# magneano/shyft

Measured on NVIDIA B200. Metric: cell-timesteps/sec (pt_gs_k run_cells), higher is better.
Workload: dtype f64

## Files before the change

### shyft_b200/csrc/sb2_capi.cu

```cuda
#include <cuda_runtime.h>

#include <cstdio>
#include <cstdlib>
#include <cstring>
#include <map>
#include <mutex>
#include <memory>
#include <string>
#include <type_traits>
#include <vector>

#include "../../include/shyft_b200.h"
#include "sb2_host.hpp"
#include "sb2_interp.cuh"
#include "sb2_ptgsk.cuh"
#include "sb2_hbv.cuh"
#include "sb2_ptssk.cuh"
#include "sb2_pthpsk.cuh"
#include "sb2_routing.cuh"
#include <nvtx3/nvToolsExt.h>
#include "sb2_unit.cuh"
#include "sb2_goal.cuh"
#include "sb2_stats.cuh"

// ... 209 lines not shown
};

inline int grid_for(int64_t n, int block) { return int((n + block - 1) / block); }

}

#define SB2_HBV_UNIT_STEPS 64
#define SB2_DENSE_TILE_COMPACT 32

struct sb2_model {
    int stack = 0, device = 0;
    cudaStream_t stream = 0;
    std::string err;
    int64_t n = 0;
    std::vector<sb2_geo_cell> geo;
    std::vector<int64_t> cix_of_cell, cix_to_cid;
    std::map<int64_t, int64_t> cid_to_cix;
    int n_param = 0, n_state = 0;
    std::vector<double> region_param;
    std::map<int64_t, std::vector<double>> catch_param;
    bool param_dirty = true;
    std::vector<uint8_t> catchment_filter;
    bool filter_dirty = true;
    DevArray<double> d_x, d_y, d_z, d_area, d_glacier, d_lake, d_reservoir, d_forest, d_slope;
    DevArray<int32_t> d_pset;
    DevArray<uint8_t> d_active;
    DevArray<PtgskParam> d_ptgsk_params;
    DevArray<HbvParam> d_hbv_params;
    DevArray<SskParam> d_ssk_params;
    DevArray<HpsParam> d_hps_params;
    DevArray<double> d_state, d_initial_state;
    bool has_initial = false;
    int64_t t0 = 0, dt = 0, T = 0;
    DevArray<int2> d_doy_soy;
    std::vector<double> h_prior_gradient;
    DevArray<double> d_prior_gradient;
    DevArray<double> d_forcing[SB2_N_FORCING];
    int64_t forcing_first = 0, forcing_rows = 0;
    Source src[SB2_N_FORCING];
    sb2_interpolation_parameter ip{};
    bool ip_valid = false;
    IdwPlan idw[SB2_N_FORCING];
    std::vector<std::unique_ptr<BtkOps>> btk_cache;
    DevArray<double> d_btk_kbuf, d_btk_beta, d_btk_resid;
    bool force_sparse_idw = false;
    int collect_bits = SB2_COLLECT_DISCHARGE;
    DevArray<double> d_resp[SB2_N_RESPONSE], d_st[SB2_N_STATE_SERIES];
    int64_t out_first = 0, out_rows = 0;
    int64_t ran_first = 0, ran_steps = 0;
    DevArray<double> d_cq, d_cc;
    DevArray<int32_t> d_slot, d_cat_ptr, d_cat_slots;
    int64_t n_slots = 0;
    DevArray<double> d_partial;
    DevArray<double> d_scr[5];
    DevArray<int> d_tickets;
    int partial_steps = 0;
    DevArray<int> d_error_flag, d_scan_flag;
    std::vector<double> rivers;
    std::unique_ptr<RoutingPlan> route;
    DevArray<double> d_rlocal, d_rup, d_rout;
    bool rlocal_valid = false, rnet_valid = false;
    DevArray<double> d_qhist;
    int64_t qhist_rows = 0;
    struct Target {
        std::vector<double> obs;
        int64_t t0 = 0, dt = 0;
        std::vector<int64_t> cids;
        int64_t river_id = 0;
        double scale_factor = 1.0;
        int calc_mode = 0, property = 0;
        double s_r = 1.0, s_a = 1.0, s_b = 1.0;
        DevArray<double> d_obs, d_series;
        DevArray<int32_t> d_cix;
        bool aligned = true;
        std::vector<int64_t> points;
        DevArray<int64_t> d_points;
        DevArray<double> d_projected, d_scale;
    };
    std::vector<std::unique_ptr<Target>> targets;
    DevArray<int32_t> d_cell_ptr, d_cell_of_catch;
    DevArray<int64_t> d_axis_t;
    DevArray<int32_t> d_one_zero;
    int64_t launches = 0;
    float last_step_ms = 0.f, last_interp_ms = 0.f;
    cudaEvent_t ev[4] = {nullptr, nullptr, nullptr, nullptr};

    int64_t n_catch() const { return int64_t(cix_to_cid.size()); }
    void use_device() const { CUDA_OK(cudaSetDevice(device)); }
};

namespace {

template <class F>
int guarded(sb2_model* m, F&& f) {
    try {
        if (!m) throw Error("null model");
        m->use_device();
        f();
        return 0;
    } catch (const std::exception& e) {
        if (m) m->err = e.what();
        return 1;
    }
}
template <class F>
int guarded_c(const sb2_model* m, F&& f) { return guarded(const_cast<sb2_model*>(m), f); }

// ... 133 lines not shown
    const PtgskParam* ptgsk_members = nullptr;
    const HbvParam* hbv_members = nullptr;
    const HpsParam* hps_members = nullptr;
    double* state = nullptr;
    double* partial = nullptr;
    double *cq = nullptr, *cc = nullptr;
    DevArray<double>* scr = nullptr;
    int64_t state_stride = 0, partial_stride = 0, catch_stride = 0, scr_stride = 0;
    int* tickets = nullptr;
    bool series = false;
};

void launch_step_chunk(sb2_model* m, const StepTarget& t, int64_t s0, int chunk, bool collect_end_state) {
    const int64_t n = m->n;
    const unsigned ne = unsigned(t.members);
    const bool gsk = m->stack == SB2_PT_GS_K;
    const int collect = t.series ? m->collect_bits : 0;
    const bool upar = m->catch_param.empty() && !t.ptgsk_members && !t.hbv_members && !t.hps_members;
    const int groups = step_groups(m);
    const bool split = use_time_split(int64_t(groups) * t.members);
    const int unit_steps = split ? (gsk ? SB2_UNIT_STEPS : SB2_HBV_UNIT_STEPS) : 0;
    const int n_slices = split ? grid_for(chunk, unit_steps) : 1;
    auto zero_tickets = [&] {
        if (split) CUDA_OK(cudaMemsetAsync(t.tickets, 0, size_t(t.members) * (1 + groups) * sizeof(int), m->stream));
    };
    auto common = [&](auto& a) {
        const double dt_seconds = double(m->dt) / 1e6;
        a.n_cells = n;
        a.area = m->d_area.p; a.glacier = m->d_glacier.p; a.lake = m->d_lake.p; a.reservoir = m->d_reservoir.p;
        a.pset = m->d_pset.p; a.active = m->d_active.p; a.state = t.state;
        for (int v = 0; v < 5; ++v) a.f[v] = m->d_forcing[v].p + (s0 - m->forcing_first) * n;
        a.n_steps = chunk; a.first_step = s0;
        a.dt_seconds = dt_seconds; a.dt_hours = dt_seconds / 3600.0; a.dt_us = double(m->dt);
        fill_dopri_products(a.dt_hours, a.dtb);
        if (t.series) {
            for (size_t r = 0; r < std::size(a.resp); ++r) a.resp[r] = m->d_resp[r].p;
            for (size_t s = 0; s < std::size(a.st); ++s) a.st[s] = m->d_st[s].p;
            a.out_first_step = m->out_first;
        }
        a.collect_end_state = collect_end_state ? 1 : 0;
        a.slot = m->d_slot.p; a.partial = t.partial; a.n_slots = m->n_slots; a.error_flag = m->d_error_flag.p;
        a.unit_steps = unit_steps; a.tickets = t.tickets; a.progress = t.tickets + t.members;
    };
    if (gsk) {
        PtgskRunArgs a{};
        common(a);
        a.z = m->d_z.p; a.forest = m->d_forest.p; a.params = m->d_ptgsk_params.p;
        a.bb0 = 0.98 * 5.670373e-8 * sb_pow4(273.15);
        a.inv_dt_seconds = make_inv_divisor(a.dt_seconds);
        a.inv_dt_us = make_inv_divisor(a.dt_us);
        a.par0 = make_ptgsk_param(m->region_param.data(), param_dt(m));
        a.day_sec_of_year = m->d_doy_soy.p;
        a.ens_params = t.ptgsk_members; a.ens_state_stride = t.state_stride; a.ens_partial_stride = t.partial_stride;
        for (int k = 0; k < 5; ++k) a.scr[k] = t.scr[k].p;
        a.ens_scr_stride = t.scr_stride;
        const dim3 ga((unsigned)grid_for(n, SB2_BLOCK_A), (unsigned)grid_for(chunk, SB2_STEPS_A), ne);
        const dim3 gb((unsigned)(grid_for(n, SB2_BLOCK_B) * n_slices), ne), gc((unsigned)(grid_for(n, SB2_BLOCK_C) * n_slices), ne);
        nvtxRangePushA("A forcing_terms");
        if (upar) ptgsk_forcing_terms_kernel<true><<<ga, SB2_BLOCK_A, SB2_MTAB_BYTES, m->stream>>>(a);
        else ptgsk_forcing_terms_kernel<false><<<ga, SB2_BLOCK_A, SB2_MTAB_BYTES, m->stream>>>(a);
        nvtxRangePop();
        zero_tickets();
        nvtxRangePushA("B snow");
        switch (collect & 14) {
#define SB2_CASE(B) case B: if (upar) ptgsk_snow_kernel<B, true><<<gb, SB2_BLOCK_B, SB2_MTAB_BYTES, m->stream>>>(a); \
                            else ptgsk_snow_kernel<B, false><<<gb, SB2_BLOCK_B, SB2_MTAB_BYTES, m->stream>>>(a); break;
            SB2_CASE(0) SB2_CASE(2) SB2_CASE(4) SB2_CASE(6) SB2_CASE(8) SB2_CASE(10) SB2_CASE(12) SB2_CASE(14)
#undef SB2_CASE
        }
        nvtxRangePop();
        zero_tickets();
        nvtxRangePushA("C response");
        switch (collect & 13) {
#define SB2_CASE(B) case B: if (upar) ptgsk_response_kernel<B, true><<<gc, SB2_BLOCK_C, SB2_MTAB_BYTES, m->stream>>>(a); \
                            else ptgsk_response_kernel<B, false><<<gc, SB2_BLOCK_C, SB2_MTAB_BYTES, m->stream>>>(a); break;
            SB2_CASE(0) SB2_CASE(1) SB2_CASE(4) SB2_CASE(5) SB2_CASE(8) SB2_CASE(9) SB2_CASE(12) SB2_CASE(13)
#undef SB2_CASE
        }
        nvtxRangePop();
        m->launches += 3;
    } else {
        const dim3 grid((unsigned)(groups * n_slices), ne);
        zero_tickets();
        if (m->stack == SB2_PT_SS_K) {
            SskRunArgs a{};
            common(a);
            a.params = m->d_ssk_params.p;
            a.inv_dt_hours = make_inv_divisor(a.dt_hours);
            a.step_in_days = a.dt_seconds / 86400.0;
            a.collect = collect & 15;
            ptssk_run_kernel<<<grid, SB2_BLOCK, SB2_MTAB_BYTES, m->stream>>>(a);
        } else if (m->stack == SB2_PT_HPS_K) {
            HpsRunArgs a{};
            common(a);
            a.params = m->d_hps_params.p;
            a.bb0 = 0.98 * 5.670373e-8 * sb_pow4(273.15);
            a.inv_dt_seconds = make_inv_divisor(a.dt_seconds);
            a.ens_params = t.hps_members; a.ens_state_stride = t.state_stride; a.ens_partial_stride = t.partial_stride;
            a.collect = collect & 15;
            if (t.hps_members) pthpsk_run_kernel<true><<<grid, SB2_BLOCK, SB2_MTAB_BYTES, m->stream>>>(a);
            else pthpsk_run_kernel<false><<<grid, SB2_BLOCK, SB2_MTAB_BYTES, m->stream>>>(a);
        } else {
            HbvRunArgs a{};
            common(a);
            a.params = m->d_hbv_params.p;
            a.inv_dt_hours = make_inv_divisor(a.dt_hours);
            a.step_in_days = a.dt_seconds / 86400.0;
// ... 482 lines not shown
            const int r = t.property == SB2_TARGET_SNOW_COVERED_AREA ? SB2_R_SNOW_SCA : SB2_R_SNOW_SWE;
            if (!m->d_resp[r].p || m->out_first != 0 || m->out_rows != m->T) throw Error(r == SB2_R_SNOW_SCA ? "resource collector doesn't have snow_sca" : "resource collector doesn't have snow_swe");
            std::vector<int32_t> cells;
            for (int64_t i = 0; i < m->n; ++i)
                for (auto cid : t.cids)
                    if (m->geo[i].catchment_id == cid) { cells.push_back(int32_t(i)); break; }
            std::vector<int32_t> ptr{0, int32_t(cells.size())};
            DevArray<int32_t> d_ptr, d_cells;
            d_ptr.upload(ptr, m->stream);
            d_cells.upload(cells, m->stream);
            t.d_series.resize(size_t(m->T));
            catchment_area_mean_kernel<<<grid_for(m->T, 256), 256, 0, m->stream>>>(m->d_resp[r].p, m->d_area.p, d_ptr.p, d_cells.p, 1, m->T, m->n,
                                                                                  t.d_series.p);
            CUDA_OK(cudaGetLastError());
            ++m->launches;
            CUDA_OK(cudaStreamSynchronize(m->stream));
        } else if (t.property == SB2_TARGET_ROUTED_DISCHARGE) {
            std::vector<double> out(size_t(m->T));
            if (sb2_river_flows(m, t.river_id, 0, m->T, nullptr, nullptr, out.data()) != 0) throw Error(m->err);
            t.d_series.upload(out, m->stream);
            CUDA_OK(cudaStreamSynchronize(m->stream));
        }
    }
}

double evaluate_goal_single(sb2_model* m) {
    prepare_snow_and_routed_targets(m);
    std::vector<GoalTarget> gt;
    build_goal_targets(m, gt, m->d_cq.p, m->d_cc.p, 0);
    DevArray<GoalTarget> d_gt;
    DevArray<double> d_out;
    d_gt.upload(gt, m->stream);
    d_out.resize(gt.size());
    goal_kernel<<<dim3((unsigned)gt.size(), 1), 256, 0, m->stream>>>(d_gt.p, int(gt.size()), d_out.p);
    CUDA_OK(cudaGetLastError());
    ++m->launches;
    std::vector<double> partial(gt.size());
    CUDA_OK(cudaMemcpyAsync(partial.data(), d_out.p, partial.size() * sizeof(double), cudaMemcpyDeviceToHost, m->stream));
    CUDA_OK(cudaStreamSynchronize(m->stream));
    return combine_goal(m, partial.data());
}

void goal_batch(sb2_model* m, int64_t n_sets, const double* P, double* goals) {
    sync_parameters(m);
    sync_filter(m);
    const bool gsk = m->stack == SB2_PT_GS_K;
    const int64_t n = m->n, T = m->T, nc = m->n_catch();
    const size_t state_sz = size_t(m->n_state) * n;
    const size_t per_member = state_sz * 8 + size_t(T) * nc * 16;
    const int64_t E = std::max<int64_t>(1, std::min<int64_t>(std::min<int64_t>(n_sets, 65535), int64_t((12ULL << 30) / per_member)));
    int64_t ps = std::min<int64_t>(T, int64_t((1ULL << 30) / (size_t(E) * m->n_slots * 16)));
    if (gsk) ps = std::min<int64_t>(ps, std::max<int64_t>(8, int64_t((4ULL << 30) / (size_t(E) * n * 40))));
    ps = std::max<int64_t>(1, ps);
    DevArray<double> d_state, d_partial, d_cq, d_cc, d_out, d_scr[5];
    if (gsk)
        for (auto& b : d_scr) b.resize(size_t(E) * ps * n);
    DevArray<int> d_tickets;
    d_tickets.resize(size_t(E) * (1 + step_groups(m)));
    DevArray<PtgskParam> d_par;
    DevArray<HbvParam> d_hbv_par;
    DevArray<HpsParam> d_hps_par;
    DevArray<GoalTarget> d_gt;
    d_state.resize(size_t(E) * state_sz);
    d_partial.resize(size_t(E) * ps * m->n_slots * 2);
    d_cq.resize(size_t(E) * T * nc);
    d_cc.resize(size_t(E) * T * nc);
    d_out.resize(size_t(E) * m->targets.size());
    std::vector<GoalTarget> gt;
    build_goal_targets(m, gt, d_cq.p, d_cc.p, T * nc);
    d_gt.upload(gt, m->stream);
    StepTarget t;
    t.state = d_state.p; t.partial = d_partial.p; t.cq = d_cq.p; t.cc = d_cc.p; t.scr = d_scr;
    t.state_stride = int64_t(state_sz); t.partial_stride = ps * m->n_slots * 2; t.catch_stride = T * nc; t.scr_stride = ps * n;
    t.tickets = d_tickets.p;
    std::vector<double> partial(size_t(E) * gt.size());
    for (int64_t e0 = 0; e0 < n_sets; e0 += E) {
        const int64_t ne = std::min<int64_t>(E, n_sets - e0);
        std::vector<const double*> sets;
        for (int64_t e = 0; e < ne; ++e) sets.push_back(P + (e0 + e) * m->n_param);
        if (gsk) { upload_params(m, sets, d_par); t.ptgsk_members = d_par.p; }
        else if (m->stack == SB2_PT_HPS_K) { upload_params(m, sets, d_hps_par); t.hps_members = d_hps_par.p; }
        else { upload_params(m, sets, d_hbv_par); t.hbv_members = d_hbv_par.p; }
        t.members = int(ne);
        for (int64_t e = 0; e < ne; ++e)
            CUDA_OK(cudaMemcpyAsync(d_state.p + e * state_sz, m->d_initial_state.p, state_sz * sizeof(double), cudaMemcpyDeviceToDevice, m->stream));
        for (int64_t done = 0; done < T; done += ps) launch_step_chunk(m, t, done, int(std::min<int64_t>(ps, T - done)), false);
        goal_kernel<<<dim3((unsigned)gt.size(), (unsigned)ne), 256, 0, m->stream>>>(d_gt.p, int(gt.size()), d_out.p);
        CUDA_OK(cudaGetLastError());
        ++m->launches;
        CUDA_OK(cudaMemcpyAsync(partial.data(), d_out.p, size_t(ne) * gt.size() * sizeof(double), cudaMemcpyDeviceToHost, m->stream));
        CUDA_OK(cudaStreamSynchronize(m->stream));
        for (int64_t e = 0; e < ne; ++e) goals[e0 + e] = combine_goal(m, partial.data() + e * gt.size());
    }
    check_device_errors(m);
}

std::vector<uint8_t> stat_selection(const sb2_model* m, const int64_t* indexes, int n_indexes, int scope) {
    if (m->n == 0) throw Error("no cells to make statistics on");
    std::vector<uint8_t> sel(size_t(m->n), n_indexes == 0 ? 1 : 0);
    if (n_indexes == 0) return sel;
    if (!indexes) throw Error("null index list");
    if (scope == SB2_SCOPE_CELL_IX) {
        for (int k = 0; k < n_indexes; ++k) {
            const int64_t cid = indexes[k];
            if (cid < 0 || cid > m->n)
                throw Error("Supplied cell index reference " + std::to_string(cid) + " is ouside valid range 0 .." + std::to_string(m->n));
            if (cid < m->n) sel[size_t(cid)] = 1;
// ... 1175 lines not shown
```

### shyft_b200/csrc/sb2_ptgsk.cuh

```cuda
#pragma once
#include <stdint.h>

#include "sb2_math.cuh"

namespace sb2 {

struct PtgskParam {
    double c1, c2, c3;
    double ae_scale_factor;
    double tx, wind_scale, max_water, wind_const, fast_albedo_decay_rate, slow_albedo_decay_rate, surface_magnitude, max_albedo,
        min_albedo, snowfall_reset_depth, snow_cv, glacier_albedo;
    double p_corr_scale_factor;
    double snow_cv_forest_factor, snow_cv_altitude_factor;
    double pt_albedo, pt_alpha;
    double initial_bare_ground_fraction;
    double gm_dtf, gm_direct_response;
    double reservoir_direct_response_fraction;
    double slow_albedo_decay_step;
    double fast_albedo_decay_step;
    int32_t winter_end_day_of_year;
    int32_t n_winter_days;
    int32_t calculate_iso_pot_energy;
    int32_t pad_;
    InvDivisor inv_snowfall_reset_depth, inv_one_minus_y0, inv_max_water, inv_ae_scale;
};

enum : int { ERR_KIRCHNER_STEP = 1 };

struct PtgskRunArgs {
    int64_t n_cells;
    const double* __restrict__ z;
    const double* __restrict__ area;
    const double* __restrict__ glacier;
    const double* __restrict__ lake;
    const double* __restrict__ reservoir;
    const double* __restrict__ forest;
    const int32_t* __restrict__ pset;
    const uint8_t* __restrict__ active;
    const PtgskParam* __restrict__ params;
    double* __restrict__ state;
    const double* __restrict__ f[5];
    int n_steps;
    int64_t first_step;
    double dt_seconds;
    double dt_hours;
    double dt_us;
    double bb0;
    InvDivisor inv_dt_seconds, inv_dt_us;
    double dtb[26];
    PtgskParam par0;
    const int2* __restrict__ day_sec_of_year;
    double* __restrict__ resp[8];
    double* __restrict__ st[9];
    int64_t out_first_step;
    int collect_end_state;
    const int32_t* __restrict__ slot;
    double* __restrict__ partial;
    int64_t n_slots;
    int* __restrict__ error_flag;
    const PtgskParam* __restrict__ ens_params;
    int64_t ens_state_stride, ens_partial_stride;
    double* __restrict__ scr[5];
    int64_t ens_scr_stride;
    int unit_steps;
    int* __restrict__ tickets;
    int* __restrict__ progress;
};
enum : int { SCR_POT = 0, SCR_LW = 1, SCR_TADD = 2, SCR_OUTFLOW = 3, SCR_SCA = 4 };

#define SB2_BLOCK 32

struct GsState { double albedo, lwc, surface_heat, alpha, sdc_melt_mean, acc_melt, iso_pot_energy, temp_swe; };
struct GsCache {
    double k_alpha, k_scale, k_acc, k_lwc, k_tswe;
    double storage, sca;
    double lg_key, lg_val;
};
__device__ __forceinline__ void gs_cache_clear(GsCache& c) {
    c.k_alpha = nan_(); c.lg_key = nan_();
    c.k_scale = c.k_acc = c.k_lwc = c.k_tswe = 0.0;
    c.storage = c.sca = c.lg_val = 0.0;
}
__device__ __forceinline__ bool gs_cache_hit(GsCache& c, double alpha, double scale, double acc, double lwc, double tswe) {
    return alpha == c.k_alpha && scale == c.k_scale && acc == c.k_acc && lwc == c.k_lwc && tswe == c.k_tswe;
}
__device__ __forceinline__ void gs_cache_store(GsCache& c, double alpha, double scale, double acc, double lwc, double tswe, double storage, double sca) {
    c.k_alpha = alpha; c.k_scale = scale; c.k_acc = acc; c.k_lwc = lwc; c.k_tswe = tswe;
    c.storage = storage; c.sca = sca;
}

enum : int { K_VP_A = 0, K_VP_B, K_VP_C, K_VP_D, K_VP_E, K_VP_F, K_VP_G, K_VP_H, K_LW, K_LW_EXP, K_SST_A, K_SST_B, K_TURB_A, K_TURB_B, K_TURB_C,
             K_SURF_A, K_SURF_B, K_KELVIN, K_PT_CK1, K_PT_PSYCR, K_PT_BOLZ, K_PT_CK2_NEG, K_PT_CK2_POS, K_PT_CK3_NEG, K_PT_CK3_POS, K_PT_EATM_A,
             K_PT_EATM_EXP, K_PT_EATM_B, K_PT_EMIS, K_MMH_M3S, K_TOL, K_EPS_ABS, K_EPS_REL, K_Q_MIN, K_GM, K_PHYS_N };
__constant__ double kPhysC[K_PHYS_N] = {33.864, 7.38e-3, 0.8072, 1.9e-5, 1.8, 1.316e-3, 9.72e-3, 4.2e-5, 0.98 * 5.670373e-8, 6.87e-2, 1.16, 2.09, 1.7, 6.12, 6.132,
                                        0.103, 0.186, 273.15, 0.610780, 0.066, 0.0000000567, 17.84362, 17.08085, 245.425, 234.175, 1.24,
                                        0.143, 0.85, 0.98, 1 / (3600.0 * 1000.0), 1.0e-10, 1.0e-7, 1.0e-8, 0.00001, 0.001 / 86400.0};
#define SB2_K(name) kPhysC[name]
__device__ __forceinline__ double mmh_to_m3s(double mmh, double area) { return area * mmh * SB2_K(K_MMH_M3S); }
__device__ __forceinline__ double m3s_to_mmh(double m3s, double area) { return m3s / (SB2_K(K_MMH_M3S) * area); }

__device__ __forceinline__ double gs_calc_q(double a, double b, double z, double lg_a, double lg_a1) {
    const double x = z / b;
    return a * b * gamma_p<true>(a + 1.0, x, lg_a1) + z * (1.0 - gamma_p<true>(a, x, lg_a));
}

__device__ __noinline__ double gs_corr_lwc(double z1, double a1, double b1, double a2, double b2) {
    const double Q1 = gs_calc_q(a1, b1, z1, sb_lgamma<true>(a1), sb_lgamma<true>(a1 + 1.0));
    const double lg_a2 = sb_lgamma<true>(a2), lg_a21 = sb_lgamma<true>(a2 + 1.0);
    auto f = [&](double z) {
        const double x = z / b2;
        double p1 = 0.0, p0 = 0.0;
        if (x == inf_()) p1 = p0 = 1.0;
        else if (x > 0.0) {
            const double lx = sb_log<true>(x);
            const double pre1 = sb_exp<true>((a2 + 1.0) * lx - x - lg_a21), pre0 = sb_exp<true>(a2 * lx - x - lg_a2);
            p1 = gamma_p_with_prefix(a2 + 1.0, x, pre1);
            p0 = gamma_p_with_prefix(a2, x, pre0);
        }
        const double d = (a2 * b2 * p1 + z * (1.0 - p0)) - Q1;
        return d * d;
    };
// ... 59 lines not shown
    if (lambda <= 0.0) {
        swe = m;
        sca = 1.0 - y0;
    } else if (lambda / scale > 1.3 * shape + 20.0) {
        swe = sca = 0.0;
        return;
    } else {
        const double x = lambda / scale;
        if (shape != lg_key) { lg_key = shape; lg_val = sb_lgamma<true>(shape); }
        lg = lg_val;
        have_lg = true;
        const double pre = gamma_prefix<true>(shape, x, lg);
        y = (x > 0.0) ? gamma_p_with_prefix(shape, x, pre) : 0.0;
        y1 = y - pre / shape;
        swe = m * (1.0 - y1) - lambda * (1 - y);
        sca = (1.0 - y) * (1.0 - y0);
    }
    if (lwd > m) swe *= 1.0 + max_water_frac;
    else if (lwd > 0.0) {
        const double sat = div_by(lwd, inv_mwf);
        const double x = sat / scale;
        if (!have_lg) {
            if (shape != lg_key) { lg_key = shape; lg_val = sb_lgamma<true>(shape); }
            lg = lg_val;
        }
        const double pre = gamma_prefix<true>(shape, x, lg);
        const double ssa = (x == inf_()) ? 1.0 : gamma_p_with_prefix(shape, x, pre);
        const double ssa1 = ssa - pre / shape;
        const double liqwat = max_water_frac * (m * (ssa1 - y1) + sat * (1.0 - ssa) - lambda * (1.0 - y));
        swe += liqwat;
    }
    swe += temp_swe;
    swe *= 1.0 - y0;
}

__device__ __forceinline__ void gs_reset_snow_pack(double& sca, double& lwc, double& alpha, double& sdc_melt_mean, double& acc_melt,
                                                   double& temp_swe, double storage, const PtgskParam& p) {
    if (storage > 1.0e-10) {
        sca = 1.0 - p.initial_bare_ground_fraction;
        sdc_melt_mean = storage / sca;
    } else {
        sca = sdc_melt_mean = 0.0;
    }
    alpha = 1.0 / (p.snow_cv * p.snow_cv);
    temp_swe = lwc = 0.0;
    acc_melt = -1.0;
}

__device__ __forceinline__ double gs_vapour_pressure(double T, double rel_hum) {
    double vapour_pressure = SB2_K(K_VP_A) * (sb_pow8(SB2_K(K_VP_B) * T + SB2_K(K_VP_C)) - SB2_K(K_VP_D) * fabs(SB2_K(K_VP_E) * T + 48.0) + SB2_K(K_VP_F)) * rel_hum;
    if (T < 0.0) vapour_pressure *= 1.0 + SB2_K(K_VP_G) * T + SB2_K(K_VP_H) * T * T;
    return vapour_pressure;
}
__device__ __forceinline__ void gs_energy_terms(const PtgskParam& p, double BB0, double T, double wind_speed, double rel_hum, double& lw, double& tadd) {
    const double tol = SB2_K(K_TOL);
    const double T_k = T + SB2_K(K_KELVIN);
    const double turb = p.wind_scale * wind_speed + p.wind_const;
    const double vapour_pressure = gs_vapour_pressure(T, rel_hum);
    lw = SB2_K(K_LW) * sb_pow_flat<true>(vapour_pressure / T_k, 6.87e-2) * sb_pow4(T_k);
    const double sst = dmin(0.0, SB2_K(K_SST_A) * T - SB2_K(K_SST_B));
    if (sst > -tol) tadd = turb * (T + SB2_K(K_TURB_A) * (vapour_pressure - SB2_K(K_TURB_B))) - BB0;
    else tadd = turb * (T - sst + SB2_K(K_TURB_A) * (vapour_pressure - SB2_K(K_TURB_C) * sb_exp_flat<true>(SB2_K(K_SURF_A) * T - SB2_K(K_SURF_B)))) - SB2_K(K_LW) * sb_pow4(sst + SB2_K(K_KELVIN));
}

struct GsStepConst { InvDivisor inv_dt_seconds, inv_dt_us; };
__device__ __forceinline__ void gs_step_core(GsState& s, GsCache& cache, double& r_sca, double& r_storage, double& r_outflow, const PtgskParam& p, int doy,
                                             int sec_of_year, double dt_seconds, double dt_us, const GsStepConst& k, double BB0, double T, double rad,
                                             double prec_mm_h, double lw, double tadd, const double* __restrict__ f_wind_speed, const double* __restrict__ f_rel_hum,
                                             int64_t f_offset, const InvDivisor& inv_cv2) {
    const double tol = SB2_K(K_TOL);
    const double melt_heat = 333660.0, water_heat = 4180.0, ice_heat = 2050.0;
    double sdc_melt_mean = s.sdc_melt_mean;
    double acc_melt = s.acc_melt;
    double iso_pot_energy = s.iso_pot_energy;
    const InvDivisor k_usec_per_hour = make_inv_divisor(3600000000.0), k_melt_heat = make_inv_divisor(333660.0);
    const double prec = div_by(prec_mm_h * dt_us, k_usec_per_hour);

    if (doy == p.winter_end_day_of_year) acc_melt = iso_pot_energy = 0.0;

    double snow, rain;
    if (T < p.tx) { snow = prec; rain = 0.0; }
    else { snow = 0.0; rain = prec; }

    if (snow < tol && sdc_melt_mean < tol && acc_melt < 0.0) {
        s.albedo = p.max_albedo;
        s.surface_heat = 0.0;
        s.iso_pot_energy = 0.0;
        r_sca = 0.0;
        r_storage = 0.0;
        r_outflow = prec_mm_h;
        return;
    }
    double albedo = s.albedo, lwc = s.lwc, surface_heat = s.surface_heat, alpha = s.alpha, temp_swe = s.temp_swe;
    double sca = 0.0, storage = 0.0, outflow = 0.0;

    const double min_albedo = p.min_albedo;
    const double max_albedo = p.max_albedo;
    const double albedo_range = max_albedo - min_albedo;

    if (snow > tol) albedo += div_by(snow * albedo_range, p.inv_snowfall_reset_depth);
    else {
        if (T < 0.0) albedo -= p.slow_albedo_decay_step;
        else albedo = min_albedo + p.fast_albedo_decay_step * (albedo - min_albedo);
    }
    albedo = dmax(dmin(albedo, max_albedo), min_albedo);

    double effect = rad * (1.0 - albedo);
    effect += lw;

    if (T > 0.0 && snow < tol) effect += div_by(rain * T * water_heat, k.inv_dt_seconds);
    if (T <= 0.0 && rain < tol) effect += div_by(snow * T * ice_heat, k.inv_dt_seconds);

    if (p.calculate_iso_pot_energy) {
        const double wind_speed = f_wind_speed[f_offset], rel_hum = f_rel_hum[f_offset];
        const double turb = p.wind_scale * wind_speed + p.wind_const;
        const double iso_effect = effect - BB0 + turb * (T + 1.7 * (gs_vapour_pressure(T, rel_hum) - 6.12));
        iso_pot_energy += div_by(iso_effect * dt_seconds, k_melt_heat);
    }

    const double sst = dmin(0.0, 1.16 * T - 2.09);
    effect += tadd;

    double delta_sh = -surface_heat;
    surface_heat = p.surface_magnitude * ice_heat * sst * 0.5;
    delta_sh += surface_heat;

    double energy = effect * dt_seconds;
    if (delta_sh > 0.0) energy -= delta_sh;

    double potential_melt = dmax(0.0, div_by(energy, k_melt_heat));

    double sdc_scale = sdc_melt_mean / alpha;
    const double y0 = p.initial_bare_ground_fraction;
    if (gs_cache_hit(cache, alpha, sdc_scale, acc_melt, lwc, temp_swe)) {
        storage = cache.storage;
        sca = cache.sca;
    } else {
        gs_calc_snow_state(alpha, sdc_scale, y0, acc_melt, lwc, p.inv_max_water, temp_swe, storage, sca, cache.lg_key, cache.lg_val);
        gs_cache_store(cache, alpha, sdc_scale, acc_melt, lwc, temp_swe, storage, sca);
    }
    const double start_storage_value = storage;

    if (acc_melt < 0.0) {
        if (snow < tol) snow = 0.0;
        else {
            const double alpha_prev = alpha;
            const double sdc_scale_prev = sdc_scale;
            const double sdc_snow = div_by(snow, p.inv_one_minus_y0);
            alpha = (sdc_melt_mean * alpha + div_by(sdc_snow, inv_cv2)) / (sdc_snow + sdc_melt_mean);
            sdc_melt_mean += sdc_snow;
            sdc_scale = sdc_melt_mean / alpha;
            if (lwc > 0.0 && sdc_snow > 0.01 * sdc_melt_mean) {
                double z1 = div_by(lwc, p.inv_max_water);
                z1 = gs_corr_lwc(z1, alpha_prev, sdc_scale_prev > 0.0 ? sdc_scale_prev : sdc_scale, alpha, sdc_scale);
                lwc = z1 * p.max_water;
                gs_calc_snow_state(alpha, sdc_scale, y0, acc_melt, lwc, p.inv_max_water, temp_swe, storage, sca, cache.lg_key, cache.lg_val);
            }
        }
        lwc += rain;
        if (sdc_melt_mean <= potential_melt) {
            storage = 0.0;
            gs_reset_snow_pack(sca, lwc, alpha, sdc_melt_mean, acc_melt, temp_swe, storage, p);
            sdc_scale = 0.0;
        } else if (potential_melt > 0.0) {
            sdc_melt_mean -= potential_melt;
            lwc += potential_melt;
            alpha = dmax(0.1, sdc_melt_mean / sdc_scale);
            if (alpha > inv_cv2.y) alpha = inv_cv2.y;
            sdc_scale = sdc_melt_mean / alpha;
        }
    } else {
        temp_swe += div_by(snow, p.inv_one_minus_y0);
        if (temp_swe > 0.0) {
            const double melt = dmin(temp_swe, potential_melt);
// ... 329 lines not shown
}

struct LaneSlot {
    unsigned lane;
    bool head;
    int slot;
};
template <class ARGS>
__device__ __forceinline__ LaneSlot lane_slot(const ARGS& a, const double* partial, int64_t cc, bool in_range, unsigned lane) {
    LaneSlot s{lane, false, -1};
    if (partial != nullptr) {
        s.slot = in_range ? a.slot[cc] : -1;
        const int prev = __shfl_up_sync(0xffffffffu, s.slot, 1);
        s.head = in_range && (lane == 0 || prev != s.slot);
    }
    return s;
}
__device__ __forceinline__ void slot_sum_store(double q, double charge, const LaneSlot& s, double* partial, int64_t po) {
    double v0 = q, v1 = charge;
#pragma unroll
    for (int off = 1; off < 32; off <<= 1) {
        const double o0 = __shfl_down_sync(0xffffffffu, v0, off);
        const double o1 = __shfl_down_sync(0xffffffffu, v1, off);
        const int os = __shfl_down_sync(0xffffffffu, s.slot, off);
        if (s.lane + off < 32 && os == s.slot) { v0 += o0; v1 += o1; }
    }
    if (s.head) {
        double* dst = partial + po;
        dst[0] = v0;
        dst[1] = v1;
    }
}

#define SB2_BLOCK_A 128
#define SB2_STEPS_A 8
#define SB2_BLOCK_B 32
#define SB2_MINBLOCKS_B 16
#define SB2_UNIT_STEPS 128
#define SB2_BLOCK_C 32
#define SB2_MINBLOCKS_C 16

#define SB2_MINBLOCKS_A 8
template <bool UPAR>
__global__ void __launch_bounds__(SB2_BLOCK_A, SB2_MINBLOCKS_A) ptgsk_forcing_terms_kernel(const __grid_constant__ PtgskRunArgs a) {
    sb_math_stage_tables();
    const int64_t c = (int64_t)blockIdx.x * blockDim.x + threadIdx.x;
    if (c >= a.n_cells) return;
    if (a.active != nullptr && a.active[c] == 0) return;
    const int ens = UPAR ? 0 : blockIdx.z;
    const PtgskParam& p = UPAR ? a.par0 : ((a.ens_params != nullptr && a.pset[c] == 0) ? a.ens_params[ens] : a.params[a.pset[c]]);
    const double pt_albedo = p.pt_albedo, pt_alpha = p.pt_alpha;
    const int64_t n = a.n_cells;
    double* __restrict__ s_pot = a.scr[SCR_POT] + (int64_t)ens * a.ens_scr_stride;
    double* __restrict__ s_lw = a.scr[SCR_LW] + (int64_t)ens * a.ens_scr_stride;
    double* __restrict__ s_tadd = a.scr[SCR_TADD] + (int64_t)ens * a.ens_scr_stride;
    const int i0 = blockIdx.y * SB2_STEPS_A;
    const int i1 = min(i0 + SB2_STEPS_A, a.n_steps);
    int64_t o = (int64_t)i0 * n + c;
    double f_t = a.f[0][o], f_r = a.f[2][o], f_w = a.f[3][o], f_h = a.f[4][o];
#pragma unroll 2
    for (int i = i0; i < i1; ++i, o += n) {
        const double temp = f_t, rad = f_r, wind = f_w, rel_hum = f_h;
        if (i + 1 < i1) { const int64_t o1 = o + n; f_t = a.f[0][o1]; f_r = a.f[2][o1]; f_w = a.f[3][o1]; f_h = a.f[4][o1]; }
        double lw, tadd;
        gs_energy_terms(p, a.bb0, temp, wind, rel_hum, lw, tadd);
        s_pot[o] = pt_potential_evapotranspiration(pt_albedo, pt_alpha, temp, rad, rel_hum) * 3600.0;
        s_lw[o] = lw;
        s_tadd[o] = tadd;
    }
}

template <int COLLECT, bool UPAR>
__global__ void __launch_bounds__(SB2_BLOCK_B, SB2_MINBLOCKS_B) ptgsk_snow_kernel(const __grid_constant__ PtgskRunArgs a) {
    sb_math_stage_tables();
    const int ens = UPAR ? 0 : blockIdx.y;
    const StepSlice sl = step_slice_begin(a, ens);
    const int i_begin = sl.i_begin, i_end = sl.i_end;
    const int64_t c = sl.group * blockDim.x + threadIdx.x;
    const bool live = c < a.n_cells && (a.active == nullptr || a.active[c] != 0);
    if (live) {
    const PtgskParam& p = UPAR ? a.par0 : ((a.ens_params != nullptr && a.pset[c] == 0) ? a.ens_params[ens] : a.params[a.pset[c]]);
    const int64_t n = a.n_cells;
    const double* __restrict__ s_lw = a.scr[SCR_LW] + (int64_t)ens * a.ens_scr_stride;
    const double* __restrict__ s_tadd = a.scr[SCR_TADD] + (int64_t)ens * a.ens_scr_stride;
    double* __restrict__ s_outflow = a.scr[SCR_OUTFLOW] + (int64_t)ens * a.ens_scr_stride;
    double* __restrict__ s_sca = a.scr[SCR_SCA] + (int64_t)ens * a.ens_scr_stride;
    const double altitude = a.z[c], cell_area_m2 = a.area[c], forest_fraction = a.forest[c];
    const double snow_storage_fraction = 1.0 - a.lake[c] - a.reservoir[c];
    const double snow_cv = p.snow_cv + forest_fraction * p.snow_cv_forest_factor + altitude * p.snow_cv_altitude_factor;
    const InvDivisor inv_cv2 = make_inv_divisor(snow_cv * snow_cv);
    const GsStepConst gk{a.inv_dt_seconds, a.inv_dt_us};
    double* __restrict__ state = a.state + (int64_t)ens * a.ens_state_stride;
    GsState gs;
    gs.albedo = __ldcg(state + 0 * n + c); gs.lwc = __ldcg(state + 1 * n + c); gs.surface_heat = __ldcg(state + 2 * n + c);
    gs.alpha = __ldcg(state + 3 * n + c); gs.sdc_melt_mean = __ldcg(state + 4 * n + c); gs.acc_melt = __ldcg(state + 5 * n + c);
    gs.iso_pot_energy = __ldcg(state + 6 * n + c); gs.temp_swe = __ldcg(state + 7 * n + c);
    GsCache cache;
    gs_cache_clear(cache);
    auto collect_state = [&](int64_t orow) {
        a.st[1][orow] = gs.albedo;
        a.st[2][orow] = gs.lwc * snow_storage_fraction;
        a.st[3][orow] = gs.surface_heat;
        a.st[4][orow] = gs.alpha;
        a.st[5][orow] = gs.sdc_melt_mean;
        a.st[6][orow] = gs.acc_melt;
        a.st[7][orow] = gs.iso_pot_energy;
        a.st[8][orow] = gs.temp_swe * snow_storage_fraction;
    };
    int64_t o = (int64_t)i_begin * n + c;
    const int64_t out_shift = (a.first_step - a.out_first_step) * n;
    const int2* __restrict__ ds_row = a.day_sec_of_year + a.first_step;
    double f_t = a.f[0][o], f_p = a.f[1][o], f_r = a.f[2][o], f_lw = s_lw[o], f_ta = s_tadd[o];
    int2 f_ds = ds_row[i_begin];
    for (int i = i_begin; i < i_end; ++i, o += n) {
        const double temp = f_t, prec = f_p * p.p_corr_scale_factor, rad = f_r, lw = f_lw, tadd = f_ta;
        const int2 ds = f_ds;
        if (i + 1 < i_end) {
            f_ds = ds_row[i + 1];
            const int64_t o1 = o + n;
            f_t = a.f[0][o1]; f_p = a.f[1][o1]; f_r = a.f[2][o1]; f_lw = s_lw[o1]; f_ta = s_tadd[o1];
        }
        if (i + SB2_PREFETCH_AHEAD < a.n_steps) {
            const int64_t o2 = o + SB2_PREFETCH_AHEAD * n;
            prefetch_l1(a.f[0] + o2); prefetch_l1(a.f[1] + o2); prefetch_l1(a.f[2] + o2); prefetch_l1(s_lw + o2); prefetch_l1(s_tadd + o2);
        }
        const int64_t orow = o + out_shift;
        if (COLLECT & 8) collect_state(orow);
        double sca, storage, outflow;
        gs_step_core(gs, cache, sca, storage, outflow, p, ds.x, ds.y, a.dt_seconds, a.dt_us, gk, a.bb0, temp, rad, prec, lw, tadd, a.f[3],
                     a.f[4], o, inv_cv2);
        s_outflow[o] = outflow;
        s_sca[o] = sca;
        if (COLLECT & 2) { a.resp[2][orow] = sca; a.resp[3][orow] = storage * snow_storage_fraction; }
        if (COLLECT & 4) a.resp[4][orow] = mmh_to_m3s(outflow * snow_storage_fraction, cell_area_m2);
    }
    if ((COLLECT & 8) && a.collect_end_state && i_end == a.n_steps) collect_state((a.first_step + a.n_steps - a.out_first_step) * n + c);
    state[0 * n + c] = gs.albedo; state[1 * n + c] = gs.lwc; state[2 * n + c] = gs.surface_heat; state[3 * n + c] = gs.alpha;
    state[4 * n + c] = gs.sdc_melt_mean; state[5 * n + c] = gs.acc_melt; state[6 * n + c] = gs.iso_pot_energy;
    state[7 * n + c] = gs.temp_swe;
    }
    step_slice_publish(sl);
}

template <int COLLECT, bool UPAR>
__global__ void __launch_bounds__(SB2_BLOCK_C, SB2_MINBLOCKS_C) ptgsk_response_kernel(const __grid_constant__ PtgskRunArgs a) {
    sb_math_stage_tables();
    const int ens = UPAR ? 0 : blockIdx.y;
    const StepSlice sl = step_slice_begin(a, ens);
    const int i_begin = sl.i_begin, i_end = sl.i_end;
    const int64_t c = sl.group * blockDim.x + threadIdx.x;
    const bool in_range = c < a.n_cells;
    const int64_t cc = in_range ? c : a.n_cells - 1;
    const bool active = in_range && (a.active == nullptr || a.active[cc] != 0);
    const unsigned lane = threadIdx.x & 31u;
    const PtgskParam& p = UPAR ? a.par0 : ((a.ens_params != nullptr && a.pset[cc] == 0) ? a.ens_params[ens] : a.params[a.pset[cc]]);
    double* __restrict__ state = a.state + (int64_t)ens * a.ens_state_stride;
    double* __restrict__ partial = a.partial != nullptr ? a.partial + (int64_t)ens * a.ens_partial_stride : nullptr;
    const double* __restrict__ s_pot = a.scr[SCR_POT] + (int64_t)ens * a.ens_scr_stride;
    const double* __restrict__ s_outflow = a.scr[SCR_OUTFLOW] + (int64_t)ens * a.ens_scr_stride;
    const double* __restrict__ s_sca = a.scr[SCR_SCA] + (int64_t)ens * a.ens_scr_stride;
    __shared__ double cst[14][SB2_BLOCK_C];
#define SB2_CST(k) (((volatile double*)cst[k])[threadIdx.x])
    {
        const double area = a.area[cc], gf = a.glacier[cc], lake = a.lake[cc], reservoir = a.reservoir[cc];
        const double gmd = p.gm_direct_response;
        const double drf = gf * gmd + reservoir * p.reservoir_direct_response_fraction;
        cst[0][threadIdx.x] = area;
        cst[1][threadIdx.x] = gf;
        cst[2][threadIdx.x] = gmd;
        cst[3][threadIdx.x] = 1 - gmd;
        cst[4][threadIdx.x] = 1.0 - lake - reservoir;
        cst[5][threadIdx.x] = reservoir * (1.0 - p.reservoir_direct_response_fraction) + lake;
        cst[6][threadIdx.x] = drf;
        cst[7][threadIdx.x] = 1 - drf;
        cst[8][threadIdx.x] = area * gf;
        cst[9][threadIdx.x] = p.ae_scale_factor;
        cst[10][threadIdx.x] = p.gm_dtf;
        cst[11][threadIdx.x] = p.p_corr_scale_factor;
        cst[12][threadIdx.x] = p.inv_ae_scale.y;
        cst[13][threadIdx.x] = 1.0 / (SB2_K(K_MMH_M3S) * area);
    }
    const unsigned ae_e_lo = p.inv_ae_scale.e_lo;
    const unsigned mmh_e_lo = make_inv_divisor(SB2_K(K_MMH_M3S) * a.area[cc]).e_lo;
// ... 115 lines not shown
```

Baseline: 9.861 billion.

## Compute longwave and turbulent energy terms inside snow kernel instead of scratch buffers

```diff
diff --git a/shyft_b200/csrc/sb2_capi.cu b/shyft_b200/csrc/sb2_capi.cu
--- a/shyft_b200/csrc/sb2_capi.cu
+++ b/shyft_b200/csrc/sb2_capi.cu
@@ -285,7 +285,7 @@
     DevArray<int32_t> d_slot, d_cat_ptr, d_cat_slots;
     int64_t n_slots = 0;
     DevArray<double> d_partial;
-    DevArray<double> d_scr[5];
+    DevArray<double> d_scr[SCR_N];
     DevArray<int> d_tickets;
     int partial_steps = 0;
     DevArray<int> d_error_flag, d_scan_flag;
@@ -525,7 +525,7 @@
         a.par0 = make_ptgsk_param(m->region_param.data(), param_dt(m));
         a.day_sec_of_year = m->d_doy_soy.p;
         a.ens_params = t.ptgsk_members; a.ens_state_stride = t.state_stride; a.ens_partial_stride = t.partial_stride;
-        for (int k = 0; k < 5; ++k) a.scr[k] = t.scr[k].p;
+        for (int k = 0; k < SCR_N; ++k) a.scr[k] = t.scr[k].p;
         a.ens_scr_stride = t.scr_stride;
         const dim3 ga((unsigned)grid_for(n, SB2_BLOCK_A), (unsigned)grid_for(chunk, SB2_STEPS_A), ne);
         const dim3 gb((unsigned)(grid_for(n, SB2_BLOCK_B) * n_slices), ne), gc((unsigned)(grid_for(n, SB2_BLOCK_C) * n_slices), ne);
@@ -1114,7 +1114,7 @@
     int64_t ps = std::min<int64_t>(T, int64_t((1ULL << 30) / (size_t(E) * m->n_slots * 16)));
     if (gsk) ps = std::min<int64_t>(ps, std::max<int64_t>(8, int64_t((4ULL << 30) / (size_t(E) * n * 40))));
     ps = std::max<int64_t>(1, ps);
-    DevArray<double> d_state, d_partial, d_cq, d_cc, d_out, d_scr[5];
+    DevArray<double> d_state, d_partial, d_cq, d_cc, d_out, d_scr[SCR_N];
     if (gsk)
         for (auto& b : d_scr) b.resize(size_t(E) * ps * n);
     DevArray<int> d_tickets;
diff --git a/shyft_b200/csrc/sb2_ptgsk.cuh b/shyft_b200/csrc/sb2_ptgsk.cuh
--- a/shyft_b200/csrc/sb2_ptgsk.cuh
+++ b/shyft_b200/csrc/sb2_ptgsk.cuh
@@ -60,13 +60,13 @@
     int* __restrict__ error_flag;
     const PtgskParam* __restrict__ ens_params;
     int64_t ens_state_stride, ens_partial_stride;
-    double* __restrict__ scr[5];
+    double* __restrict__ scr[3];
     int64_t ens_scr_stride;
     int unit_steps;
     int* __restrict__ tickets;
     int* __restrict__ progress;
 };
-enum : int { SCR_POT = 0, SCR_LW = 1, SCR_TADD = 2, SCR_OUTFLOW = 3, SCR_SCA = 4 };
+enum : int { SCR_POT = 0, SCR_OUTFLOW = 1, SCR_SCA = 2, SCR_N };
 
 #define SB2_BLOCK 32
 
@@ -232,22 +232,21 @@
     if (T < 0.0) vapour_pressure *= 1.0 + SB2_K(K_VP_G) * T + SB2_K(K_VP_H) * T * T;
     return vapour_pressure;
 }
-__device__ __forceinline__ void gs_energy_terms(const PtgskParam& p, double BB0, double T, double wind_speed, double rel_hum, double& lw, double& tadd) {
+struct GsEnergyTerms { double lw, tadd; };
+__device__ __forceinline__ GsEnergyTerms gs_energy_terms(double BB0, double T, double sst, double turb, double vapour_pressure) {
     const double tol = SB2_K(K_TOL);
     const double T_k = T + SB2_K(K_KELVIN);
-    const double turb = p.wind_scale * wind_speed + p.wind_const;
-    const double vapour_pressure = gs_vapour_pressure(T, rel_hum);
-    lw = SB2_K(K_LW) * sb_pow_flat<true>(vapour_pressure / T_k, 6.87e-2) * sb_pow4(T_k);
-    const double sst = dmin(0.0, SB2_K(K_SST_A) * T - SB2_K(K_SST_B));
-    if (sst > -tol) tadd = turb * (T + SB2_K(K_TURB_A) * (vapour_pressure - SB2_K(K_TURB_B))) - BB0;
-    else tadd = turb * (T - sst + SB2_K(K_TURB_A) * (vapour_pressure - SB2_K(K_TURB_C) * sb_exp_flat<true>(SB2_K(K_SURF_A) * T - SB2_K(K_SURF_B)))) - SB2_K(K_LW) * sb_pow4(sst + SB2_K(K_KELVIN));
+    GsEnergyTerms e;
+    e.lw = SB2_K(K_LW) * sb_pow_flat<true>(vapour_pressure / T_k, 6.87e-2) * sb_pow4(T_k);
+    if (sst > -tol) e.tadd = turb * (T + SB2_K(K_TURB_A) * (vapour_pressure - SB2_K(K_TURB_B))) - BB0;
+    else e.tadd = turb * (T - sst + SB2_K(K_TURB_A) * (vapour_pressure - SB2_K(K_TURB_C) * sb_exp_flat<true>(SB2_K(K_SURF_A) * T - SB2_K(K_SURF_B)))) - SB2_K(K_LW) * sb_pow4(sst + SB2_K(K_KELVIN));
+    return e;
 }
 
 struct GsStepConst { InvDivisor inv_dt_seconds, inv_dt_us; };
 __device__ __forceinline__ void gs_step_core(GsState& s, GsCache& cache, double& r_sca, double& r_storage, double& r_outflow, const PtgskParam& p, int doy,
                                              int sec_of_year, double dt_seconds, double dt_us, const GsStepConst& k, double BB0, double T, double rad,
-                                             double prec_mm_h, double lw, double tadd, const double* __restrict__ f_wind_speed, const double* __restrict__ f_rel_hum,
-                                             int64_t f_offset, const InvDivisor& inv_cv2) {
+                                             double prec_mm_h, double wind_speed, double rel_hum, const InvDivisor& inv_cv2) {
     const double tol = SB2_K(K_TOL);
     const double melt_heat = 333660.0, water_heat = 4180.0, ice_heat = 2050.0;
     double sdc_melt_mean = s.sdc_melt_mean;
@@ -285,21 +284,23 @@
     }
     albedo = dmax(dmin(albedo, max_albedo), min_albedo);
 
+    const double sst = dmin(0.0, SB2_K(K_SST_A) * T - SB2_K(K_SST_B));
+    const double turb = p.wind_scale * wind_speed + p.wind_const;
+    const double vapour_pressure = gs_vapour_pressure(T, rel_hum);
+    const GsEnergyTerms et = gs_energy_terms(BB0, T, sst, turb, vapour_pressure);
+
     double effect = rad * (1.0 - albedo);
-    effect += lw;
+    effect += et.lw;
 
     if (T > 0.0 && snow < tol) effect += div_by(rain * T * water_heat, k.inv_dt_seconds);
     if (T <= 0.0 && rain < tol) effect += div_by(snow * T * ice_heat, k.inv_dt_seconds);
 
     if (p.calculate_iso_pot_energy) {
-        const double wind_speed = f_wind_speed[f_offset], rel_hum = f_rel_hum[f_offset];
-        const double turb = p.wind_scale * wind_speed + p.wind_const;
-        const double iso_effect = effect - BB0 + turb * (T + 1.7 * (gs_vapour_pressure(T, rel_hum) - 6.12));
+        const double iso_effect = effect - BB0 + turb * (T + 1.7 * (vapour_pressure - 6.12));
         iso_pot_energy += div_by(iso_effect * dt_seconds, k_melt_heat);
     }
 
-    const double sst = dmin(0.0, 1.16 * T - 2.09);
-    effect += tadd;
+    effect += et.tadd;
 
     double delta_sh = -surface_heat;
     surface_heat = p.surface_magnitude * ice_heat * sst * 0.5;
@@ -735,21 +736,15 @@
     const double pt_albedo = p.pt_albedo, pt_alpha = p.pt_alpha;
     const int64_t n = a.n_cells;
     double* __restrict__ s_pot = a.scr[SCR_POT] + (int64_t)ens * a.ens_scr_stride;
-    double* __restrict__ s_lw = a.scr[SCR_LW] + (int64_t)ens * a.ens_scr_stride;
-    double* __restrict__ s_tadd = a.scr[SCR_TADD] + (int64_t)ens * a.ens_scr_stride;
     const int i0 = blockIdx.y * SB2_STEPS_A;
     const int i1 = min(i0 + SB2_STEPS_A, a.n_steps);
     int64_t o = (int64_t)i0 * n + c;
-    double f_t = a.f[0][o], f_r = a.f[2][o], f_w = a.f[3][o], f_h = a.f[4][o];
+    double f_t = a.f[0][o], f_r = a.f[2][o], f_h = a.f[4][o];
 #pragma unroll 2
     for (int i = i0; i < i1; ++i, o += n) {
-        const double temp = f_t, rad = f_r, wind = f_w, rel_hum = f_h;
-        if (i + 1 < i1) { const int64_t o1 = o + n; f_t = a.f[0][o1]; f_r = a.f[2][o1]; f_w = a.f[3][o1]; f_h = a.f[4][o1]; }
-        double lw, tadd;
-        gs_energy_terms(p, a.bb0, temp, wind, rel_hum, lw, tadd);
+        const double temp = f_t, rad = f_r, rel_hum = f_h;
+        if (i + 1 < i1) { const int64_t o1 = o + n; f_t = a.f[0][o1]; f_r = a.f[2][o1]; f_h = a.f[4][o1]; }
         s_pot[o] = pt_potential_evapotranspiration(pt_albedo, pt_alpha, temp, rad, rel_hum) * 3600.0;
-        s_lw[o] = lw;
-        s_tadd[o] = tadd;
     }
 }
 
@@ -764,8 +759,6 @@
     if (live) {
     const PtgskParam& p = UPAR ? a.par0 : ((a.ens_params != nullptr && a.pset[c] == 0) ? a.ens_params[ens] : a.params[a.pset[c]]);
     const int64_t n = a.n_cells;
-    const double* __restrict__ s_lw = a.scr[SCR_LW] + (int64_t)ens * a.ens_scr_stride;
-    const double* __restrict__ s_tadd = a.scr[SCR_TADD] + (int64_t)ens * a.ens_scr_stride;
     double* __restrict__ s_outflow = a.scr[SCR_OUTFLOW] + (int64_t)ens * a.ens_scr_stride;
     double* __restrict__ s_sca = a.scr[SCR_SCA] + (int64_t)ens * a.ens_scr_stride;
     const double altitude = a.z[c], cell_area_m2 = a.area[c], forest_fraction = a.forest[c];
@@ -793,25 +786,24 @@
     int64_t o = (int64_t)i_begin * n + c;
     const int64_t out_shift = (a.first_step - a.out_first_step) * n;
     const int2* __restrict__ ds_row = a.day_sec_of_year + a.first_step;
-    double f_t = a.f[0][o], f_p = a.f[1][o], f_r = a.f[2][o], f_lw = s_lw[o], f_ta = s_tadd[o];
+    double f_t = a.f[0][o], f_p = a.f[1][o], f_r = a.f[2][o], f_w = a.f[3][o], f_h = a.f[4][o];
     int2 f_ds = ds_row[i_begin];
     for (int i = i_begin; i < i_end; ++i, o += n) {
-        const double temp = f_t, prec = f_p * p.p_corr_scale_factor, rad = f_r, lw = f_lw, tadd = f_ta;
+        const double temp = f_t, prec = f_p * p.p_corr_scale_factor, rad = f_r, wind = f_w, rel_hum = f_h;
         const int2 ds = f_ds;
         if (i + 1 < i_end) {
             f_ds = ds_row[i + 1];
             const int64_t o1 = o + n;
-            f_t = a.f[0][o1]; f_p = a.f[1][o1]; f_r = a.f[2][o1]; f_lw = s_lw[o1]; f_ta = s_tadd[o1];
+            f_t = a.f[0][o1]; f_p = a.f[1][o1]; f_r = a.f[2][o1]; f_w = a.f[3][o1]; f_h = a.f[4][o1];
         }
         if (i + SB2_PREFETCH_AHEAD < a.n_steps) {
             const int64_t o2 = o + SB2_PREFETCH_AHEAD * n;
-            prefetch_l1(a.f[0] + o2); prefetch_l1(a.f[1] + o2); prefetch_l1(a.f[2] + o2); prefetch_l1(s_lw + o2); prefetch_l1(s_tadd + o2);
+            prefetch_l1(a.f[0] + o2); prefetch_l1(a.f[1] + o2); prefetch_l1(a.f[2] + o2); prefetch_l1(a.f[3] + o2); prefetch_l1(a.f[4] + o2);
         }
         const int64_t orow = o + out_shift;
         if (COLLECT & 8) collect_state(orow);
         double sca, storage, outflow;
-        gs_step_core(gs, cache, sca, storage, outflow, p, ds.x, ds.y, a.dt_seconds, a.dt_us, gk, a.bb0, temp, rad, prec, lw, tadd, a.f[3],
-                     a.f[4], o, inv_cv2);
+        gs_step_core(gs, cache, sca, storage, outflow, p, ds.x, ds.y, a.dt_seconds, a.dt_us, gk, a.bb0, temp, rad, prec, wind, rel_hum, inv_cv2);
         s_outflow[o] = outflow;
         s_sca[o] = sca;
         if (COLLECT & 2) { a.resp[2][orow] = sca; a.resp[3][orow] = storage * snow_storage_fraction; }
```

New measurement: 9.622 billion (median of 6 runs). -2.4%, worse.
